# pfnet-research/superpixel-align

Measured on AMD Instinct MI355X. Metric: images/sec superpixel-align labelling (1024x2048), higher is better.
Workload: dtype f32 as 2 x f16 planes, f32 accumulate

## Files before the change

superpixel-align_amd/csrc/spa_common.h:

```cpp
#pragma once
#include <hip/hip_runtime.h>
#include <stdint.h>
#include <stdio.h>
#include <string.h>

#include "../../include/spalign.h"

#define SPA_WAVE 64

void spa_set_error(const char *fmt, ...);

#define SPA_HIP(call)                                                                  \
    do {                                                                               \
        hipError_t e_ = (call);                                                        \
        if (e_ != hipSuccess) {                                                        \
            spa_set_error("%s failed: %s (%s:%d)", #call, hipGetErrorString(e_),      \
                          __FILE__, __LINE__);                                         \
            return SPA_ERR_HIP;                                                        \
        }                                                                              \
    } while (0)

#define SPA_ARG(cond)                                                                  \
    do {                                                                               \
        if (!(cond)) {                                                                 \
// ... 40 lines not shown
    WS_FZ_KEYS,
    WS_FZ_VALS,
    WS_FZ_STATE,
    WS_FZ_TMP,
    WS_STEM_WPACK,
    WS_ZERO_LINE,
    WS_RESIZE_TAB,
    WS_RESIZE_TMP,
    WS_RNG_STATE,
    WS_RNG_RING,
    WS_RNG_JBUF,
    WS_RNG_JOFF,
    WS_RUNS,
    WS_DEBUG,
    WS_SEGNET_BNPART,
    WS_SEGNET_WROT,
    WS_SEGNET_WGRAD,
    WS_SEGNET_WBF16,
    WS_SEGNET_WF16X3,
    WS_SEGNET_AMAX,
    WS_SEGNET_BNRED,
    WS_PNG_ROWS,
    WS_JPEG_INTERVALS,
    WS_COUNT
};

enum {
    PROF_RGB2LAB = 0, PROF_SLIC_ASSIGN, PROF_SLIC_UPDATE, PROF_CONNECT, PROF_STATS,
    PROF_CELL_WEIGHTS, PROF_POOL_MEAN, PROF_POOL_ANCHOR, PROF_KMEANS, PROF_PAINT,
    PROF_DRN_STEM, PROF_DRN_BIAS_ACT, PROF_DRN_CONV, PROF_DRN_CONV32, PROF_DRN_GEMM32, PROF_DRN_GEMM32_N, PROF_WINO_IN, PROF_WINO_OUT, PROF_DRN_GEMM16, PROF_DRN_GEMM16_N, PROF_DRN_CONV16, PROF_DRN_CONV16_128, PROF_DRN_CONV16_256, PROF_DRN_CONV16_1X1, PROF_DRN_CONV16_FRONT, PROF_DRN_CONV_LIGHT, PROF_SLOTS
};

struct spa_ctx {
    int device;
    int n_cu;
    uint32_t *d_status;
    unsigned status_takes;
    void *ws[WS_COUNT];
    size_t ws_bytes[WS_COUNT];
    int prof_on;
    hipEvent_t *prof_ev[PROF_SLOTS];
    int prof_cap[PROF_SLOTS], prof_used[PROF_SLOTS];
    hipStream_t aux[2];
    hipEvent_t ev_fork, ev_join[2];
    int aux_ready;
    int km_attr_done[2];
    int conn_attr_done;
    int conn_claim_ready;
    size_t conn_claim_bytes;
    int upd_wg_per_cu, upd_wg_per_cu8;
    int slic_force_general;
    int zero_line_ready, conv_attr_done, conv32_attr_done, fz_attr_done, gemm16_attr_done, gemm16s_attr_done, gemm16p_attr_done, nprng_attr_done;
    int rng_seeded;
    int ws_generation;
    int dbg_slic_ldsx;
    int convp_on;
    int wino_operands;
    int convs2_on;
    int convs2_attr_done;
    int rs_key[4], rs_ks[2];
};

#ifdef __HIPCC__
__device__ __forceinline__ unsigned spa_split16_pair(float x0, float x1, float sc, unsigned &l)
{
    unsigned h, lo;
    asm("v_fma_mixlo_f16 %0, %2, %4, 0 op_sel_hi:[0,0,0]\n\t"
        "v_fma_mixhi_f16 %0, %3, %4, 0 op_sel_hi:[0,0,0]\n\t"
        "v_fma_mixlo_f16 %1, %2, %4, -%0 op_sel_hi:[0,0,1]\n\t"
        "v_fma_mixhi_f16 %1, %3, %4, -%0 op_sel:[0,0,1] op_sel_hi:[0,0,1]"
        : "=&v"(h), "=&v"(lo) : "v"(x0), "v"(x1), "v"(sc));
    l = lo;
    return h;
}
#endif

int spa_aux_streams(spa_ctx *ctx);

void spa_prof_mark(spa_ctx *ctx, int slot, int end, hipStream_t s);
struct SpaProfScope {
    spa_ctx *c; int slot; hipStream_t s;
    SpaProfScope(spa_ctx *c_, int slot_, hipStream_t s_) : c(c_), slot(slot_), s(s_) { if (c->prof_on && slot >= 0) spa_prof_mark(c, slot, 0, s); }
    ~SpaProfScope() { if (c->prof_on && slot >= 0) spa_prof_mark(c, slot, 1, s); }
};

int spa_ws_reserve(spa_ctx *ctx, int which, size_t bytes, void **out);
void spa_zero_word(void *word, hipStream_t s);

static inline hipStream_t spa_stream(void *s) { return (hipStream_t)s; }

__device__ __forceinline__ double spa_det_log_pos(double x)
{
    unsigned long long b = (unsigned long long)__double_as_longlong(x);
    int e = (int)((b >> 52) & 0x7ff) - 1023;
    b = (b & 0x000fffffffffffffULL) | 0x3ff0000000000000ULL;
    double m = __longlong_as_double((long long)b);
    if (m > 1.4142135623730951) { m = m * 0.5; e += 1; }
    double s = (m - 1.0) / (m + 1.0);
    double z = s * s;
    double p = 1.0 / 25.0;
    p = p * z + 1.0 / 23.0;
    p = p * z + 1.0 / 21.0;
    p = p * z + 1.0 / 19.0;
    p = p * z + 1.0 / 17.0;
    p = p * z + 1.0 / 15.0;
    p = p * z + 1.0 / 13.0;
    p = p * z + 1.0 / 11.0;
    p = p * z + 1.0 / 9.0;
    p = p * z + 1.0 / 7.0;
    p = p * z + 1.0 / 5.0;
// ... 37 lines not shown
```

superpixel-align_amd/csrc/spa_convs2.hip:

```cpp
#include "spa_common.h"

typedef float s2_f4 __attribute__((ext_vector_type(4)));
typedef _Float16 s2_h8 __attribute__((ext_vector_type(8)));

#define S2_TW 32
#define S2_PW (2 * S2_TW + 1)

__device__ __forceinline__ void s2_lds_barrier()
{
    asm volatile("s_waitcnt lgkmcnt(0)\n\ts_barrier" ::: "memory");
}

template <int CIN> struct S2Geom {
    static constexpr int TH = CIN == 32 ? 4 : 2;
    static constexpr int PH = 2 * TH + 1;
    static constexpr int PITCH = 4 * CIN + 16;
    static constexpr int PATCH = PH * S2_PW * PITCH;
    static constexpr int NW = 8;
    static constexpr int NE = PH * S2_PW * (CIN / 4), NU = (NE + NW * 64 - 1) / (NW * 64);
    static constexpr int NS = CIN == 32 ? 0 : (NU < 9 ? NU : 9);
    static constexpr int LDS = PATCH + NS * NW * 1024;
    static_assert(LDS <= 160 * 1024 && PATCH % 16 == 0, "LDS of a CU");
};

template <int CIN, int NG, bool PROJ>
__global__ __launch_bounds__(S2Geom<CIN>::NW * 64) void k_conv3x3_s2_tile(const float *__restrict__ x, int B, int Hi, int Wi, int Ho, int Wo,
                                                                const unsigned short *__restrict__ wt2, const float *__restrict__ bias,
                                                                float inv_t, int relu, const unsigned *__restrict__ amax_in,
                                                                unsigned *__restrict__ amax_out, float *__restrict__ y,
                                                                float *__restrict__ y2)
{
    typedef S2Geom<CIN> G;
    constexpr int TH = G::TH, PITCH = G::PITCH, KC = CIN / 32, CS = 16 * NG;
    constexpr int NW = G::NW, S2_THREADS = NW * 64, NE = G::NE, NU = G::NU, NS = G::NS;
    constexpr bool LIGHT = CIN == 64;
    constexpr int NPH = NW / NG, ITER = TH / NPH;
    static_assert(TH % NPH == 0 && NPH * NG == NW, "rows per wave");
    extern __shared__ __attribute__((aligned(16))) char s2_patch[];
    const int tid = threadIdx.x, lane = tid & 63;
    const int wave = __builtin_amdgcn_readfirstlane(tid >> 6);
    const int frow = lane & 15, fk = lane >> 4;
    const int cg = wave % NG, ph = wave / NG;
    const int tiles_x = (Wo + S2_TW - 1) / S2_TW, tiles_y = (Ho + TH - 1) / TH;
    const int n_tiles = tiles_x * tiles_y * B;

    s2_h8 wh[9][KC], wl[9][KC], qh[KC], ql[KC];
    float4 bias_c, bias_p;
    {
        const unsigned short *wr = wt2 + (size_t)(cg * 16 + frow) * (9 * KC * 64) + 8 * fk;
#pragma unroll
        for (int tap = 0; tap < 9; ++tap)
#pragma unroll
            for (int kc = 0; kc < KC; ++kc) {
                wh[tap][kc] = *(const s2_h8 *)(wr + (tap * KC + kc) * 64);
                wl[tap][kc] = *(const s2_h8 *)(wr + (tap * KC + kc) * 64 + 32);
            }
        bias_c = bias_p = make_float4(0.f, 0.f, 0.f, 0.f);
        if (!LIGHT) bias_c = *(const float4 *)(bias + cg * 16 + 4 * fk);
        if (PROJ && !LIGHT) {
            const unsigned short *pr = wt2 + (size_t)(CS + cg * 16 + frow) * (9 * KC * 64) + 8 * fk;
#pragma unroll
// ... 16 lines not shown
    constexpr int Q = CIN / 4;
    float4 raw[NU - NS > 0 ? NU - NS : 1];
    char *const stage = s2_patch + G::PATCH + wave * 1024;
    auto patch_load = [&](int tile) {
        const int b = tile / (tiles_x * tiles_y), tr = tile - b * (tiles_x * tiles_y);
        const int ty0 = (tr / tiles_x) * TH, tx0 = (tr % tiles_x) * S2_TW;
        const float *src = x + (long long)b * Hi * Wi * CIN;
#pragma unroll
        for (int u = 0; u < NU; ++u) {
            int e = tid + u * S2_THREADS;
            e = e < NE ? e : NE - 1;
            const int pix = e / Q, q = e % Q;
            const int iy = pix / S2_PW, ix = pix - iy * S2_PW;
            const int gy = 2 * ty0 - 1 + iy, gx = 2 * tx0 - 1 + ix;
            const int cy = min(max(gy, 0), Hi - 1), cx = min(max(gx, 0), Wi - 1);
            const float *g = src + ((long long)cy * Wi + cx) * CIN + 4 * q;
            if (u < NS)
                __builtin_amdgcn_global_load_lds((const __attribute__((address_space(1))) void *)g,
                                                 (__attribute__((address_space(3))) void *)(stage + u * (NW * 1024)), 16, 0, 0);
            else raw[u - NS] = *(const float4 *)g;
        }
    };
    unsigned amx = 0;
    if ((int)blockIdx.x < n_tiles) patch_load(blockIdx.x);
    for (int tile = blockIdx.x; tile < n_tiles; tile += gridDim.x) {
        const int b = tile / (tiles_x * tiles_y), tr = tile - b * (tiles_x * tiles_y);
        const int ty0 = (tr / tiles_x) * TH, tx0 = (tr % tiles_x) * S2_TW;
        if (NS > 0) asm volatile("s_waitcnt vmcnt(0)" ::: "memory");
#pragma unroll
        for (int u = 0; u < NU; ++u) {
            const int e = tid + u * S2_THREADS;
            if (e >= NE) continue;
            const int pix = e / Q, q = e % Q;
            const int iy = pix / S2_PW, ix = pix - iy * S2_PW;
            const int gy = 2 * ty0 - 1 + iy, gx = 2 * tx0 - 1 + ix;
            const bool in = (unsigned)gy < (unsigned)Hi && (unsigned)gx < (unsigned)Wi;
            const float4 rv = u < NS ? *(const float4 *)(stage + u * (NW * 1024) + 16 * lane) : raw[u < NS ? 0 : u - NS];
            const float v0 = in ? rv.x : 0.f, v1 = in ? rv.y : 0.f, v2 = in ? rv.z : 0.f, v3 = in ? rv.w : 0.f;
            unsigned l01, l23;
            const unsigned h01 = spa_split16_pair(v0, v1, sc, l01);
            const unsigned h23 = spa_split16_pair(v2, v3, sc, l23);
            char *o = s2_patch + pix * PITCH + q * 8;
            *(uint2 *)o = make_uint2(h01, h23);
            *(uint2 *)(o + 2 * CIN) = make_uint2(l01, l23);
        }
        s2_lds_barrier();
        if (tile + (int)gridDim.x < n_tiles) patch_load(tile + (int)gridDim.x);
#pragma unroll 1
        for (int it = 0; it < ITER; ++it) {
            const int r = ph * ITER + it;
            const char *pb = s2_patch + ((2 * r) * S2_PW + 2 * frow) * PITCH + 16 * fk;
            s2_f4 c0 = {0.f, 0.f, 0.f, 0.f}, c1 = {0.f, 0.f, 0.f, 0.f}, p0 = {0.f, 0.f, 0.f, 0.f}, p1 = {0.f, 0.f, 0.f, 0.f};
            if (PROJ && LIGHT) {
                size_t off = (size_t)(CS + frow) * (9 * KC * 64) + 8 * fk + 4 * KC * 64;
                asm volatile("" : "+v"(off));
#pragma unroll
                for (int kc = 0; kc < KC; ++kc) {
                    const unsigned short *pr = wt2 + off + (size_t)(cg * 16) * (9 * KC * 64) + kc * 64;
                    qh[kc] = *(const s2_h8 *)pr;
                    ql[kc] = *(const s2_h8 *)(pr + 32);
                }
            }
#pragma unroll
            for (int dy = 0; dy < 3; ++dy)
#pragma unroll
                for (int kc = 0; kc < KC; ++kc)
#pragma unroll
                    for (int dx = 0; dx < 3; ++dx) {
                        const int tap = dy * 3 + dx;
                        const char *f = pb + (dy * S2_PW + dx) * PITCH + kc * 64;
// ... 24 lines not shown
                for (int hf = 0; hf < 2; ++hf) {
                    const int gx = tx0 + hf * 16 + frow;
                    if (gx >= Wo) continue;
                    const long long pix = ((long long)b * Ho + gy) * Wo + gx;
                    const s2_f4 a = hf ? c1 : c0;
                    if (LIGHT) {
                        bias_c = *(const float4 *)(bias + cg * 16 + 4 * fk);
                        if (PROJ) bias_p = *(const float4 *)(bias + CS + cg * 16 + 4 * fk);
                    }
                    float v0 = a[0] * unscale + bias_c.x, v1 = a[1] * unscale + bias_c.y, v2 = a[2] * unscale + bias_c.z, v3 = a[3] * unscale + bias_c.w;
                    if (relu) { v0 = fmaxf(v0, 0.f); v1 = fmaxf(v1, 0.f); v2 = fmaxf(v2, 0.f); v3 = fmaxf(v3, 0.f); }
                    *(float4 *)(y + pix * CS + cg * 16 + 4 * fk) = make_float4(v0, v1, v2, v3);
                    amx = max(max(amx, __float_as_uint(v0) & 0x7fffffffu), max(__float_as_uint(v1) & 0x7fffffffu,
                              max(__float_as_uint(v2) & 0x7fffffffu, __float_as_uint(v3) & 0x7fffffffu)));
                    if (PROJ) {
                        const s2_f4 p = hf ? p1 : p0;
                        *(float4 *)(y2 + pix * CS + cg * 16 + 4 * fk) = make_float4(p[0] * unscale + bias_p.x, p[1] * unscale + bias_p.y,
                                                                                    p[2] * unscale + bias_p.z, p[3] * unscale + bias_p.w);
                    }
                }
            }
        }
        s2_lds_barrier();
    }
    if (amax_out) {
        for (int o = 32; o > 0; o >>= 1) amx = max(amx, (unsigned)__shfl_xor((int)amx, o));
        if (lane == 0 && amx > *(volatile unsigned *)amax_out) atomicMax(amax_out, amx);
    }
}

template <int CIN, int NG, bool PROJ>
static int s2_tile_launch(spa_ctx *ctx, int bit, const float *x, int B, int Hi, int Wi, const void *wt2, float inv_t, const float *bias,
                          int relu, const void *amax_in, void *amax_out, float *y, float *y2, hipStream_t s)
{
    typedef S2Geom<CIN> G;
    constexpr int NW = G::NW;
    if (!(ctx->convs2_attr_done & bit)) {
        SPA_HIP(hipFuncSetAttribute((const void *)k_conv3x3_s2_tile<CIN, NG, PROJ>, hipFuncAttributeMaxDynamicSharedMemorySize, G::LDS));
        ctx->convs2_attr_done |= bit;
    }
    const int Ho = (Hi + 1) / 2, Wo = (Wi + 1) / 2;
    const long long n_tiles = (long long)((Wo + S2_TW - 1) / S2_TW) * ((Ho + G::TH - 1) / G::TH) * B;
    SPA_ARG(n_tiles < (1ll << 31));
    long long grid = ctx->n_cu;
    if (grid > n_tiles) grid = n_tiles;
    hipLaunchKernelGGL((k_conv3x3_s2_tile<CIN, NG, PROJ>), dim3((unsigned)grid), dim3(NW * 64), G::LDS, s, x, B, Hi, Wi, Ho, Wo,
                       (const unsigned short *)wt2, bias, inv_t, relu, (const unsigned *)amax_in, (unsigned *)amax_out, y, y2);
    SPA_LAUNCH_CHECK();
    return SPA_OK;
}

bool conv3x3_s2_tile_takes(int32_t Cin, int32_t Cout, int32_t csplit, const float *y2)
{
    if (Cin != 32 && Cin != 64) return false;
    if (y2) return (csplit == 64 || csplit == 128) && Cout == 2 * csplit;
    return csplit == 128 && Cout == 128;
}

int conv3x3_s2_tile_launch(spa_ctx *ctx, const float *x, int32_t B, int32_t Hi, int32_t Wi, int32_t Cin, const void *wt2, float inv_t,
                           int32_t csplit, const float *bias, int32_t relu, const void *amax_in, void *amax_out, float *y, float *y2,
                           hipStream_t s)
{
#define S2_GO(C, N, P, BIT) return s2_tile_launch<C, N, P>(ctx, BIT, x, B, Hi, Wi, wt2, inv_t, bias, relu, amax_in, amax_out, y, y2, s)
    if (y2) {
        if (Cin == 32 && csplit == 64) S2_GO(32, 4, true, 1);
        if (Cin == 32 && csplit == 128) S2_GO(32, 8, true, 2);
        if (Cin == 64 && csplit == 64) S2_GO(64, 4, true, 4);
        if (Cin == 64 && csplit == 128) S2_GO(64, 8, true, 8);
    } else {
        if (Cin == 32 && csplit == 128) S2_GO(32, 8, false, 16);
// ... 7 lines not shown
```

superpixel-align_amd/csrc/spa_ctx.hip:

```cpp
#include <math.h>
#include <stdarg.h>
#include <stdlib.h>

#include "spa_common.h"

static thread_local char g_err[512] = "";

void spa_set_error(const char *fmt, ...)
{
    va_list ap;
    va_start(ap, fmt);
    vsnprintf(g_err, sizeof(g_err), fmt, ap);
    va_end(ap);
}

extern "C" const char *spa_last_error(void) { return g_err; }
extern "C" int spa_version(void) { return 100; }

extern "C" int spa_ctx_create(int device, spa_ctx **out)
{
    SPA_ARG(out != nullptr);
    int n = 0;
    if (hipGetDeviceCount(&n) != hipSuccess || n <= 0) {
        spa_set_error("no HIP device visible: libspalign has no CPU fallback");
        return SPA_ERR_NOGPU;
    }
    if (device < 0) SPA_HIP(hipGetDevice(&device));
    SPA_ARG(device < n);
    SPA_HIP(hipSetDevice(device));
    hipDeviceProp_t prop;
    SPA_HIP(hipGetDeviceProperties(&prop, device));
    if (strncmp(prop.gcnArchName, "gfx950", 6) != 0) {
        spa_set_error("device %d is %s; libspalign is built for gfx950 (MI355X) only", device,
                      prop.gcnArchName);
        return SPA_ERR_NOGPU;
    }
    spa_ctx *ctx = (spa_ctx *)calloc(1, sizeof(spa_ctx));
    ctx->device = device;
    ctx->n_cu = prop.multiProcessorCount;
    if (const char *e = getenv("SPA_SLIC_GENERAL")) ctx->slic_force_general = atoi(e) != 0;
    ctx->convp_on = getenv("SPA_CONVP") ? atoi(getenv("SPA_CONVP")) != 0 : 1;
    ctx->convs2_on = 1;
    ctx->wino_operands = 2;
    SPA_HIP(hipMalloc((void **)&ctx->d_status, 32 * sizeof(uint32_t)));
    SPA_HIP(hipMemset(ctx->d_status, 0, 32 * sizeof(uint32_t)));
    *out = ctx;
    return SPA_OK;
}

extern "C" void spa_ctx_destroy(spa_ctx *ctx)
{
    if (!ctx) return;
    for (int i = 0; i < PROF_SLOTS; ++i) {
        for (int j = 0; j < ctx->prof_cap[i]; ++j) (void)hipEventDestroy(ctx->prof_ev[i][j]);
        free(ctx->prof_ev[i]);
    }
    for (int i = 0; i < WS_COUNT; ++i)
        if (ctx->ws[i]) (void)hipFree(ctx->ws[i]);
    if (ctx->d_status) (void)hipFree(ctx->d_status);
    if (ctx->aux_ready) {
        for (int i = 0; i < 2; ++i) { (void)hipStreamDestroy(ctx->aux[i]); (void)hipEventDestroy(ctx->ev_join[i]); }
        (void)hipEventDestroy(ctx->ev_fork);
    }
    free(ctx);
}

__global__ void k_zero_word(unsigned *w) { *w = 0u; }
void spa_zero_word(void *word, hipStream_t s) { hipLaunchKernelGGL(k_zero_word, dim3(1), dim3(1), 0, s, (unsigned *)word); }

int spa_ws_reserve(spa_ctx *ctx, int which, size_t bytes, void **out)
{
    if (bytes == 0) bytes = 16;
    if (ctx->ws_bytes[which] < bytes) {
        SPA_HIP(hipDeviceSynchronize());
        if (ctx->ws[which]) SPA_HIP(hipFree(ctx->ws[which]));
        ctx->ws[which] = nullptr;
        ctx->ws_bytes[which] = 0;
        size_t want = bytes + bytes / 8;
        SPA_HIP(hipMalloc(&ctx->ws[which], want));
        ctx->ws_bytes[which] = want;
        ++ctx->ws_generation;
    }
    *out = ctx->ws[which];
    return SPA_OK;
}

extern "C" int spa_status(spa_ctx *ctx, uint32_t *status_host, void *stream)
{
    SPA_ARG(ctx && status_host);
    hipStream_t s = spa_stream(stream);
    SPA_HIP(hipMemcpyAsync(status_host, ctx->d_status, sizeof(uint32_t), hipMemcpyDeviceToHost, s));
// ... 199 lines not shown
            const bool take = best[i] > dd[i];
            best[i] = take ? dd[i] : best[i];
            bl[i] = take ? jj : bl[i];
        }
        if (p0.x < 1e30f) acc0 = p0;
        if (p1.x < 1e30f) acc1 = p1;
    }
    float4 r = make_float4(best[0] + (float)bl[0], best[1] + (float)bl[1], best[2] + (float)bl[2], best[3] + (float)bl[3]);
    *(float4 *)(out + ((long long)blockIdx.x * 256 + tid) * 4) = r;
}

extern "C" int spa_debug_lds_probe(spa_ctx *ctx, float *out, int32_t n_wg, int32_t steps, int32_t mode, void *stream)
{
    SPA_ARG(ctx && out && n_wg > 0 && steps > 0 && steps <= 32 && mode >= 0 && mode <= 2);
    hipLaunchKernelGGL(k_debug_lds_probe, dim3((unsigned)n_wg), dim3(256), 0, spa_stream(stream), out, steps, mode, 0.731f);
    SPA_LAUNCH_CHECK();
    return SPA_OK;
}

extern "C" int spa_ws_generation(spa_ctx *ctx) { return ctx ? ctx->ws_generation : -1; }

extern "C" int spa_debug_set(spa_ctx *ctx, int32_t key, int32_t value)
{
    SPA_ARG(ctx && (key == 1 || key == 2 || key == 3 || key == 4) && (value == 0 || value == 1 || (key == 4 && value == 2)));
    if (key == 1) ctx->convp_on = value;
    else if (key == 4) ctx->wino_operands = value;
    else if (key == 3) ctx->convs2_on = value;
    else {
#ifdef SPA_DIAG
        ctx->dbg_slic_ldsx = value;
#else
        SPA_ARG(!"spa_debug_set key 2 (the reproducer variant of k_slic_assign) exists in diagnostic builds only: make EXTRA=-DSPA_DIAG");
#endif
    }
    return SPA_OK;
}

extern "C" int spa_debug_peek(spa_ctx *ctx, int which, size_t offset, size_t bytes, void *host)
{
    if (which == -1) which = WS_DEBUG;
    SPA_ARG(ctx && host && which >= 0 && which < WS_COUNT && offset + bytes <= ctx->ws_bytes[which]);
    SPA_HIP(hipDeviceSynchronize());
    SPA_HIP(hipMemcpy(host, (const char *)ctx->ws[which] + offset, bytes, hipMemcpyDeviceToHost));
    return SPA_OK;
}
```

superpixel-align_amd/csrc/spa_stem.hip:

```cpp
#include "spa_common.h"

#define ST_TH 16
#define ST_TW 32
#define ST_IH (ST_TH + 8)
#define ST_IW (ST_TW + 8)
#define ST_IPLANE (ST_IH * ST_IW + 8)
#define ST_LH (ST_TH + 2)
#define ST_LW (ST_TW + 2)
#define ST_LP (ST_LH * ST_LW)
#define ST_PS 17
#define ST_K0 148
#define ST_S0 (ST_K0 / 4)
#define ST_S1 (144 / 4)
#define ST_PF 8

typedef float stem_f4 __attribute__((ext_vector_type(4)));

__device__ __forceinline__ unsigned short stem_bf16(float f)
{
    const unsigned u = __float_as_uint(f);
    if ((u & 0x7fffffffu) > 0x7f800000u) return (unsigned short)((u >> 16) | 0x0040u);
    return (unsigned short)((u + 0x7fffu + ((u >> 16) & 1u)) >> 16);
}

// ... 306 lines not shown
        }
        stem_lds_barrier();
    }
}

typedef _Float16 stem_h8 __attribute__((ext_vector_type(8)));
#define SH_PW 48
#define SH_PLANE (ST_IH * SH_PW + 16)
#define SH_COPY (3 * SH_PLANE + 48)
#define SH_L0_PITCH 32
#define SH_IN_S0 4096.0f

__device__ __forceinline__ unsigned short stem_f16_bits(float f)
{
    const _Float16 h = (_Float16)f;
    return __builtin_bit_cast(unsigned short, h);
}
__device__ __forceinline__ float stem_f16_val(unsigned short b) { return (float)__builtin_bit_cast(_Float16, b); }

__global__ __launch_bounds__(256, 2) void k_drn_stem_d_f16x3(const float *__restrict__ xn, int B, int H, int W,
                                                             const unsigned short *__restrict__ wp,
                                                             const float *__restrict__ b0, const float *__restrict__ b1,
                                                             float *__restrict__ y, unsigned *__restrict__ amax_out,
                                                             float *__restrict__ y0)
{
    __shared__ __attribute__((aligned(16))) unsigned short in_h[2][SH_COPY], in_l[2][SH_COPY];
    unsigned amx = 0;
    __shared__ __attribute__((aligned(16))) unsigned short l0_s[ST_LP * SH_L0_PITCH + 64];
    const int tid = threadIdx.x, lane = tid & 63, wv = tid >> 6;
    const int m = lane & 15, g = lane >> 4;
    const long long npix = (long long)H * W;
    const int tiles_x = (W + ST_TW - 1) / ST_TW, tiles_y = (H + ST_TH - 1) / ST_TH;
    const int n_tiles = tiles_x * tiles_y * B;

    stem_h8 w0h[6], w0l[6], w1h[5], w1l[5];
#pragma unroll
    for (int s = 0; s < 6; ++s) {
        w0h[s] = *(const stem_h8 *)(wp + ((size_t)s * 64 + lane) * 8);
        w0l[s] = *(const stem_h8 *)(wp + ((size_t)(6 + s) * 64 + lane) * 8);
    }
#pragma unroll
    for (int s = 0; s < 5; ++s) {
        w1h[s] = *(const stem_h8 *)(wp + ((size_t)(12 + s) * 64 + lane) * 8);
        w1l[s] = *(const stem_h8 *)(wp + ((size_t)(17 + s) * 64 + lane) * 8);
    }
    const float *sc = (const float *)(wp + (size_t)22 * 64 * 8);
    const float unscale0 = sc[0], s1 = sc[1], unscale1 = sc[2];
    const float4 bias0 = *(const float4 *)(b0 + 4 * g), bias1 = *(const float4 *)(b1 + 4 * g);
// ... 17 lines not shown
    int eiy[NU], eix[NU], elds[NU];
#pragma unroll
    for (int u = 0; u < NU; ++u) {
        int e = tid + u * 256;
        const bool ok = e < NE;
        if (!ok) e = NE - 1;
        const int pix = e / 3, c = e - pix * 3;
        eiy[u] = pix / ST_IW; eix[u] = pix - eiy[u] * ST_IW;
        elds[u] = ok ? c * SH_PLANE + eiy[u] * SH_PW + eix[u] : -1;
        eix[u] = eix[u] * 4 + c;
    }
    auto patch_load = [&](int tile) {
        const int b = tile / (tiles_x * tiles_y), tr = tile - b * (tiles_x * tiles_y);
        const int ty0 = (tr / tiles_x) * ST_TH, tx0 = (tr % tiles_x) * ST_TW;
        const float *src = xn + (long long)b * npix * 3;
#pragma unroll
        for (int u = 0; u < NU; ++u) {
            const int gy = ty0 - 4 + eiy[u], gx = tx0 - 4 + (eix[u] >> 2);
            const int cy = min(max(gy, 0), H - 1), cx = min(max(gx, 0), W - 1);
            raw[u] = src[(unsigned)((cy * W + cx) * 3 + (eix[u] & 3))];
        }
    };
    for (int i = tid; i < SH_COPY; i += 256) { in_h[0][i] = 0; in_h[1][i] = 0; in_l[0][i] = 0; in_l[1][i] = 0; }
    if ((int)blockIdx.x < n_tiles) patch_load(blockIdx.x);
    __syncthreads();

    for (int tile = blockIdx.x; tile < n_tiles; tile += gridDim.x) {
        const int b = tile / (tiles_x * tiles_y), tr = tile - b * (tiles_x * tiles_y);
        const int ty0 = (tr / tiles_x) * ST_TH, tx0 = (tr % tiles_x) * ST_TW;
#pragma unroll
        for (int u = 0; u < NU; ++u) {
            const int ix = eix[u] >> 2;
            const int gy = ty0 - 4 + eiy[u], gx = tx0 - 4 + ix;
            const bool in = (unsigned)gy < (unsigned)H && (unsigned)gx < (unsigned)W;
            if (elds[u] >= 0) {
                const float v = in ? raw[u] * SH_IN_S0 : 0.0f;
                const unsigned short vh = stem_f16_bits(v);
                const unsigned short vl = stem_f16_bits(v - stem_f16_val(vh));
                in_h[0][elds[u]] = vh; in_l[0][elds[u]] = vl;
                if (ix >= 1) { in_h[1][elds[u] - 1] = vh; in_l[1][elds[u] - 1] = vl; }
            }
        }
        stem_lds_barrier();

        for (int t = wv; t < (ST_LP + 15) / 16; t += 4) {
            int p = t * 16 + m;
            if (p > ST_LP - 1) p = ST_LP - 1;
            const int py = p / ST_LW, px = p - py * ST_LW;
            const int boff = py * SH_PW + (px & ~1);
            const unsigned short *bh = in_h[px & 1] + boff, *bl = in_l[px & 1] + boff;
            stem_f4 acc = {0.0f, 0.0f, 0.0f, 0.0f};
#pragma unroll
            for (int s = 0; s < 6; ++s) {
                const uint32_t *qh = (const uint32_t *)(bh + goff[s]), *ql = (const uint32_t *)(bl + goff[s]);
                union { uint32_t u[4]; stem_h8 v; } fh, fl;
                fh.u[0] = qh[0]; fh.u[1] = qh[1]; fh.u[2] = qh[2]; fh.u[3] = qh[3];
                fl.u[0] = ql[0]; fl.u[1] = ql[1]; fl.u[2] = ql[2]; fl.u[3] = ql[3];
                acc = __builtin_amdgcn_mfma_f32_16x16x32_f16(w0l[s], fh.v, acc, 0, 0, 0);
                acc = __builtin_amdgcn_mfma_f32_16x16x32_f16(w0h[s], fl.v, acc, 0, 0, 0);
                acc = __builtin_amdgcn_mfma_f32_16x16x32_f16(w0h[s], fh.v, acc, 0, 0, 0);
            }
            const int q0 = t * 16 + m;
            if (q0 < ST_LP) {
                const int gy = ty0 - 1 + py, gx = tx0 - 1 + px;
                const bool in = gy >= 0 && gy < H && gx >= 0 && gx < W;
                float v[4] = {acc[0] * unscale0 + bias0.x, acc[1] * unscale0 + bias0.y, acc[2] * unscale0 + bias0.z, acc[3] * unscale0 + bias0.w};
                unsigned short vh[4], vl[4];
#pragma unroll
                for (int j = 0; j < 4; ++j) {
                    const float r = in ? fmaxf(v[j], 0.0f) * s1 : 0.0f;
                    vh[j] = stem_f16_bits(r);
                    vl[j] = stem_f16_bits(r - stem_f16_val(vh[j]));
                }
                if (y0 && in && py >= 1 && py <= ST_TH && px >= 1 && px <= ST_TW)
                    *(float4 *)(y0 + ((((long long)b * H + gy) * W + gx) * 16 + 4 * g)) =
                        make_float4(fmaxf(v[0], 0.0f), fmaxf(v[1], 0.0f), fmaxf(v[2], 0.0f), fmaxf(v[3], 0.0f));
                const int sw = (q0 << 2) & 16;
                unsigned short *o = l0_s + q0 * SH_L0_PITCH + 4 * g;
                *(uint2 *)(o + sw) = make_uint2((unsigned)vh[0] | ((unsigned)vh[1] << 16), (unsigned)vh[2] | ((unsigned)vh[3] << 16));
                *(uint2 *)(o + 16 - sw) = make_uint2((unsigned)vl[0] | ((unsigned)vl[1] << 16), (unsigned)vl[2] | ((unsigned)vl[3] << 16));
            }
        }
        stem_lds_barrier();
        if (tile + (int)gridDim.x < n_tiles) patch_load(tile + (int)gridDim.x);

        for (int t = wv; t < 32; t += 4) {
            const int row = t >> 1, col = (t & 1) * 16 + m;
            stem_f4 acc = {0.0f, 0.0f, 0.0f, 0.0f};
            const int qb = row * ST_LW + col;
#pragma unroll
            for (int s = 0; s < 5; ++s) {
                const int q = qb + l1off[s];
                const int sw = (q << 2) & 16;
                const unsigned short *lb = l0_s + q * SH_L0_PITCH + 8 * (g & 1);
                const stem_h8 fh = *(const stem_h8 *)(lb + sw);
                const stem_h8 fl = *(const stem_h8 *)(lb + 16 - sw);
                acc = __builtin_amdgcn_mfma_f32_16x16x32_f16(w1l[s], fh, acc, 0, 0, 0);
                acc = __builtin_amdgcn_mfma_f32_16x16x32_f16(w1h[s], fl, acc, 0, 0, 0);
                acc = __builtin_amdgcn_mfma_f32_16x16x32_f16(w1h[s], fh, acc, 0, 0, 0);
            }
            const int gy = ty0 + row, gx = tx0 + col;
            if (gy < H && gx < W) {
                const float4 o = make_float4(fmaxf(acc[0] * unscale1 + bias1.x, 0.0f), fmaxf(acc[1] * unscale1 + bias1.y, 0.0f),
                                             fmaxf(acc[2] * unscale1 + bias1.z, 0.0f), fmaxf(acc[3] * unscale1 + bias1.w, 0.0f));
                *(float4 *)(y + ((((long long)b * H + gy) * W + gx) * 16 + 4 * g)) = o;
                amx = max(amx, max(max(__float_as_uint(o.x), __float_as_uint(o.y)), max(__float_as_uint(o.z), __float_as_uint(o.w))));
            }
        }
        stem_lds_barrier();
    }
    if (amax_out) {
        for (int o = 32; o > 0; o >>= 1) amx = max(amx, (unsigned)__shfl_xor((int)amx, o));
        if (lane == 0 && amx > *(volatile unsigned *)amax_out) atomicMax(amax_out, amx);
    }
}

#define L2_TH 4
#define L2_TW 32
#define L2_PH (2 * L2_TH + 1)
#define L2_PW (2 * L2_TW + 1)
#define L2_PITCH 40

__global__ __launch_bounds__(256, 2) void k_drn_layer2_f16x3(const float *__restrict__ x, int B, int H, int W, int Ho, int Wo,
                                                             const unsigned short *__restrict__ wp, const float *__restrict__ bias,
                                                             float inv_t, const unsigned *__restrict__ amax_in,
                                                             unsigned *__restrict__ amax_out, float *__restrict__ y)
{
    __shared__ __attribute__((aligned(16))) unsigned short patch[L2_PH * L2_PW * L2_PITCH + 64];
    const int tid = threadIdx.x, lane = tid & 63, wv = tid >> 6;
    const int m = lane & 15, g = lane >> 4;
    const int tiles_x = (Wo + L2_TW - 1) / L2_TW, tiles_y = (Ho + L2_TH - 1) / L2_TH;
    const int n_tiles = tiles_x * tiles_y * B;
    stem_h8 wh[2][5], wl[2][5];
#pragma unroll
    for (int ct = 0; ct < 2; ++ct)
#pragma unroll
        for (int s = 0; s < 5; ++s) {
            wh[ct][s] = *(const stem_h8 *)(wp + ((size_t)((ct * 2 + 0) * 5 + s) * 64 + lane) * 8);
            wl[ct][s] = *(const stem_h8 *)(wp + ((size_t)((ct * 2 + 1) * 5 + s) * 64 + lane) * 8);
        }
    float sc, unscale;
    {
        const unsigned bits = *amax_in;
        int e = (int)(bits >> 23) - 127;
        e = bits == 0u ? 0 : (e < -100 ? -100 : (e > 100 ? 100 : e));
        sc = __uint_as_float((unsigned)(127 + 14 - e) << 23);
        unscale = __uint_as_float((unsigned)(127 - 14 + e) << 23) * inv_t;
    }
    const float4 bias_lo = *(const float4 *)(bias + 4 * g), bias_hi = *(const float4 *)(bias + 16 + 4 * g);
    int toff[5];
#pragma unroll
// ... 6 lines not shown
    float4 raw[NU];
    int epix[NU], eq[NU];
#pragma unroll
    for (int u = 0; u < NU; ++u) {
        int e = tid + u * 256;
        if (e >= NE) e = -1;
        epix[u] = e < 0 ? -1 : e >> 2;
        eq[u] = e & 3;
    }
    auto patch_load = [&](int tile) {
        const int b = tile / (tiles_x * tiles_y), tr = tile - b * (tiles_x * tiles_y);
        const int ty0 = (tr / tiles_x) * L2_TH, tx0 = (tr % tiles_x) * L2_TW;
        const float *src = x + (long long)b * H * W * 16;
#pragma unroll
        for (int u = 0; u < NU; ++u) {
            const int pix = epix[u] < 0 ? 0 : epix[u];
            const int iy = pix / L2_PW, ix = pix - iy * L2_PW;
            const int gy = 2 * ty0 - 1 + iy, gx = 2 * tx0 - 1 + ix;
            const int cy = min(max(gy, 0), H - 1), cx = min(max(gx, 0), W - 1);
            raw[u] = *(const float4 *)(src + ((long long)cy * W + cx) * 16 + 4 * eq[u]);
        }
    };
    unsigned amx = 0;
    if ((int)blockIdx.x < n_tiles) patch_load(blockIdx.x);
    for (int tile = blockIdx.x; tile < n_tiles; tile += gridDim.x) {
        const int b = tile / (tiles_x * tiles_y), tr = tile - b * (tiles_x * tiles_y);
        const int ty0 = (tr / tiles_x) * L2_TH, tx0 = (tr % tiles_x) * L2_TW;
#pragma unroll
        for (int u = 0; u < NU; ++u) {
            if (epix[u] < 0) continue;
            const int iy = epix[u] / L2_PW, ix = epix[u] - iy * L2_PW;
            const int gy = 2 * ty0 - 1 + iy, gx = 2 * tx0 - 1 + ix;
            const bool in = (unsigned)gy < (unsigned)H && (unsigned)gx < (unsigned)W;
            const float v[4] = {in ? raw[u].x * sc : 0.f, in ? raw[u].y * sc : 0.f, in ? raw[u].z * sc : 0.f, in ? raw[u].w * sc : 0.f};
            unsigned short vh[4], vl[4];
#pragma unroll
            for (int j = 0; j < 4; ++j) { vh[j] = stem_f16_bits(v[j]); vl[j] = stem_f16_bits(v[j] - stem_f16_val(vh[j])); }
            unsigned short *o = patch + epix[u] * L2_PITCH + 4 * eq[u];
            *(uint2 *)o = make_uint2((unsigned)vh[0] | ((unsigned)vh[1] << 16), (unsigned)vh[2] | ((unsigned)vh[3] << 16));
            *(uint2 *)(o + 16) = make_uint2((unsigned)vl[0] | ((unsigned)vl[1] << 16), (unsigned)vl[2] | ((unsigned)vl[3] << 16));
        }
        stem_lds_barrier();
        if (tile + (int)gridDim.x < n_tiles) patch_load(tile + (int)gridDim.x);
        for (int t = wv; t < (L2_TH * L2_TW) / 16; t += 4) {
            const int row = t >> 1, col = (t & 1) * 16 + m;
            const unsigned short *pb = patch + ((2 * row) * L2_PW + 2 * col) * L2_PITCH;
            stem_f4 a0 = {0.f, 0.f, 0.f, 0.f}, a1 = {0.f, 0.f, 0.f, 0.f};
#pragma unroll
            for (int s = 0; s < 5; ++s) {
                const stem_h8 fh = *(const stem_h8 *)(pb + toff[s]);
                const stem_h8 fl = *(const stem_h8 *)(pb + toff[s] + 16);
                a0 = __builtin_amdgcn_mfma_f32_16x16x32_f16(wl[0][s], fh, a0, 0, 0, 0);
                a1 = __builtin_amdgcn_mfma_f32_16x16x32_f16(wl[1][s], fh, a1, 0, 0, 0);
                a0 = __builtin_amdgcn_mfma_f32_16x16x32_f16(wh[0][s], fl, a0, 0, 0, 0);
                a1 = __builtin_amdgcn_mfma_f32_16x16x32_f16(wh[1][s], fl, a1, 0, 0, 0);
                a0 = __builtin_amdgcn_mfma_f32_16x16x32_f16(wh[0][s], fh, a0, 0, 0, 0);
                a1 = __builtin_amdgcn_mfma_f32_16x16x32_f16(wh[1][s], fh, a1, 0, 0, 0);
            }
            const int gy = ty0 + row, gx = tx0 + col;
            if (gy < Ho && gx < Wo) {
                const float4 o0 = make_float4(fmaxf(a0[0] * unscale + bias_lo.x, 0.f), fmaxf(a0[1] * unscale + bias_lo.y, 0.f),
                                              fmaxf(a0[2] * unscale + bias_lo.z, 0.f), fmaxf(a0[3] * unscale + bias_lo.w, 0.f));
                const float4 o1 = make_float4(fmaxf(a1[0] * unscale + bias_hi.x, 0.f), fmaxf(a1[1] * unscale + bias_hi.y, 0.f),
                                              fmaxf(a1[2] * unscale + bias_hi.z, 0.f), fmaxf(a1[3] * unscale + bias_hi.w, 0.f));
                float *o = y + (((long long)b * Ho + gy) * Wo + gx) * 32 + 4 * g;
                *(float4 *)o = o0;
                *(float4 *)(o + 16) = o1;
                amx = max(amx, max(max(__float_as_uint(o0.x), __float_as_uint(o0.y)), max(__float_as_uint(o0.z), __float_as_uint(o0.w))));
                amx = max(amx, max(max(__float_as_uint(o1.x), __float_as_uint(o1.y)), max(__float_as_uint(o1.z), __float_as_uint(o1.w))));
            }
        }
        stem_lds_barrier();
    }
    if (amax_out) {
        for (int o = 32; o > 0; o >>= 1) amx = max(amx, (unsigned)__shfl_xor((int)amx, o));
        if (lane == 0 && amx > *(volatile unsigned *)amax_out) atomicMax(amax_out, amx);
    }
}

extern "C" int spa_drn_layer2_f16s(spa_ctx *ctx, const float *x, int32_t B, int32_t H, int32_t W, const void *wp, float inv_t,
                                   const float *bias, const void *amax_in, void *amax_out, float *y, void *stream)
{
    SPA_ARG(ctx && x && wp && bias && amax_in && y && B > 0 && H > 0 && W > 0 && inv_t > 0.f);
    SPA_ARG((((uintptr_t)x | (uintptr_t)wp | (uintptr_t)bias | (uintptr_t)y) & 15) == 0);
    hipStream_t s = spa_stream(stream);
    if (amax_out) spa_zero_word(amax_out, s);
    const int Ho = (H + 1) / 2, Wo = (W + 1) / 2;
    const long long n_tiles = (long long)((Wo + L2_TW - 1) / L2_TW) * ((Ho + L2_TH - 1) / L2_TH) * B;
    SPA_ARG(n_tiles < (1ll << 31));
    SpaProfScope prof_(ctx, PROF_DRN_CONV16_FRONT, s);
    long long grid = 3ll * ctx->n_cu;
    if (grid > n_tiles) grid = n_tiles;
    hipLaunchKernelGGL(k_drn_layer2_f16x3, dim3((unsigned)grid), dim3(256), 0, s, x, B, H, W, Ho, Wo, (const unsigned short *)wp, bias,
                       inv_t, (const unsigned *)amax_in, (unsigned *)amax_out, y);
    SPA_LAUNCH_CHECK();
    return SPA_OK;
}

__global__ __launch_bounds__(256) void k_drn_layer2_f32(const float *__restrict__ x, int B, int H, int W, int Ho, int Wo,
                                                       const float4 *__restrict__ w9, const float *__restrict__ bias, float *__restrict__ y)
{
    __shared__ float4 lw[9 * 16 * 8];
    for (int i = threadIdx.x; i < 9 * 16 * 8; i += 256) lw[i] = w9[i];
    __syncthreads();
    const long long id = (long long)blockIdx.x * 256 + threadIdx.x;
    if (id >= (long long)B * Ho * Wo) return;
    const int xo = (int)(id % Wo);
    const long long t = id / Wo;
    const int yo = (int)(t % Ho), b = (int)(t / Ho);
    typedef float l2f2 __attribute__((ext_vector_type(2)));
    l2f2 acc[16];
#pragma unroll
    for (int n = 0; n < 16; ++n) acc[n] = (l2f2){bias[2 * n], bias[2 * n + 1]};
    for (int tap = 0; tap < 9; ++tap) {
        const int yy = 2 * yo - 1 + tap / 3, xx = 2 * xo - 1 + tap % 3;
        if (yy < 0 || yy >= H || xx < 0 || xx >= W) continue;
        const float4 *px = (const float4 *)(x + (((long long)b * H + yy) * W + xx) * 16);
// ... 155 lines not shown
        if ((rc = spa_ws_reserve(ctx, WS_STEM_WPACK, (size_t)11 * 64 * 8 * 2, (void **)&wp)) != SPA_OK) return rc;
        hipLaunchKernelGGL(k_stem_pack_bf16, dim3(11), dim3(64), 0, spa_stream(stream), w0, w1, wp);
        unsigned short *xb = (unsigned short *)xn_scratch;
        if (!xb && (rc = spa_ws_reserve(ctx, WS_STEM_IN, (size_t)B * H * W * 3 * sizeof(float), (void **)&xb)) != SPA_OK) return rc;
        if ((rc = spa_drn_normalise(ctx, x, B, H, W, xb, 1, mean3_host, std3_host, stream)) != SPA_OK) return rc;
        hipLaunchKernelGGL(k_drn_stem_d_bf16, dim3((unsigned)grid), dim3(256), 0, spa_stream(stream), (const unsigned short *)xb, B,
                           H, W, (const unsigned short *)wp, b0, (const unsigned short *)(wp + 6 * 64 * 8), b1,
                           (unsigned short *)y, (unsigned short *)y0);
        SPA_LAUNCH_CHECK();
        return SPA_OK;
    }
    float *xn = xn_scratch;
    if (!xn) rc = spa_ws_reserve(ctx, WS_STEM_IN, (size_t)B * H * W * 3 * sizeof(float), (void **)&xn);
    if (rc != SPA_OK) return rc;
    rc = spa_drn_normalise(ctx, x, B, H, W, xn, 0, mean3_host, std3_host, stream);
    if (rc != SPA_OK) return rc;
    if (out_dtype == 2) {
        if (amax_out) spa_zero_word(amax_out, spa_stream(stream));
        unsigned short *wp;
        if ((rc = spa_ws_reserve(ctx, WS_STEM_WPACK, (size_t)22 * 64 * 8 * 2 + 16, (void **)&wp)) != SPA_OK) return rc;
        hipLaunchKernelGGL(k_stem_pack_f16, dim3(23), dim3(64), 0, spa_stream(stream), w0, b0, w1, wp);
        long long g2 = 2ll * ctx->n_cu;
        if (g2 > n_tiles) g2 = n_tiles;
        hipLaunchKernelGGL(k_drn_stem_d_f16x3, dim3((unsigned)g2), dim3(256), 0, spa_stream(stream), (const float *)xn, B, H, W,
                           (const unsigned short *)wp, b0, b1, (float *)y, (unsigned *)amax_out, y0);
        SPA_LAUNCH_CHECK();
        return SPA_OK;
    }
    hipLaunchKernelGGL(k_drn_stem_d, dim3((unsigned)grid), dim3(256), 0, spa_stream(stream), (const float *)xn, B, H, W,
                       w0, b0, w1, b1, y, (int)out_dtype);
    SPA_LAUNCH_CHECK();
    return SPA_OK;
}
```

superpixel-align_amd/drn.py:

```python
import collections
import gc
import math
import os
from functools import partial

import numpy as np
import torch
import torch.nn as nn
import torch.nn.functional as F

IMAGENET_MEAN = (0.485, 0.456, 0.406)
IMAGENET_STD = (0.229, 0.224, 0.225)
CHAINER_BN_EPS = 2e-5

_PLANS = {
    'drn_c_26': ('C', (1, 1, 2, 2, 2, 2, 1, 1)),
    'drn_d_22': ('D', (1, 1, 2, 2, 2, 2, 1, 1)),
}
_CHANNELS = (16, 32, 64, 128, 256, 512, 512, 512)


def _conv(cin, cout, k, stride=1, dilation=1):
    pad = dilation * (k // 2)
    return nn.Conv2d(cin, cout, k, stride=stride, padding=pad, dilation=dilation, bias=False)
# ... 46 lines not shown
        for i in range(3):
            c[i] += v[i]


def _graph_wanted(x):
    mode = os.environ.get('SPA_DRN_GRAPH', '')
    if mode == '0' or not x.is_cuda:
        return False
    if mode == '1':
        return True
    return x.shape[0] * x.shape[2] * x.shape[3] <= int(os.environ.get('SPA_DRN_GRAPH_PIXELS', str(4 << 20)))


F32, BF16 = torch.float32, torch.bfloat16
Flags = collections.namedtuple('Flags', 'split_gemm own_conv own_conv32 winograd bf16_light wino_min_cin debug')
Layer = collections.namedtuple('Layer', 'cin cout k stride dilation folded families')
Call = collections.namedtuple('Call', 'dtype B H W gpu layout residual relu')


def _flags():
    E, eng = _EPILOGUE, _EPILOGUE['engine']
    return Flags(E['split_gemm'], E['own_conv'], E['own_conv32'], E['winograd'], os.environ.get('SPA_BF16_LIGHT', '1') != '0',
                 int(os.environ.get('SPA_WINO_MIN_CIN', '256')),
                 None if eng is None else (eng.debug_get(1, 1), eng.debug_get(3, 1), eng.debug_get(4, 2)))


def _nhwc(*tensors):
    return all(t is None or t.is_contiguous(memory_format=torch.channels_last) for t in tensors)


def _layer(conv, bn, holder=None):
    return Layer(conv.in_channels, conv.out_channels, conv.kernel_size[0], conv.stride[0], conv.dilation[0],
                 isinstance(bn, nn.Identity) and conv.bias is not None, tuple(getattr(holder or conv, '_spa_ops', ())))


def _call(x, residual, relu):
    return Call(x.dtype, x.shape[0], x.shape[2], x.shape[3], _EPILOGUE['engine'] is not None and x.is_cuda, _nhwc(x, residual),
                residual is not None, relu)


def _row_fills(W, bn):
    return -(-W // bn) * bn <= 1.25 * W


def _out(n, stride):
    return -(-n // stride)

# ... 676 lines not shown
```

Measured before the change: 443.7.

## Replace static tile striding with atomic work-stealing queue in front conv kernels

```diff
diff --git a/superpixel-align_amd/csrc/spa_common.h b/superpixel-align_amd/csrc/spa_common.h
--- a/superpixel-align_amd/csrc/spa_common.h
+++ b/superpixel-align_amd/csrc/spa_common.h
@@ -86,6 +86,7 @@
     WS_SEGNET_BNRED,
     WS_PNG_ROWS,
     WS_JPEG_INTERVALS,
+    WS_TILE_QUEUE,
     WS_COUNT
 };
 
@@ -122,6 +123,8 @@
     int wino_operands;
     int convs2_on;
     int convs2_attr_done;
+    int tile_queue_on;
+    unsigned tile_queue_launches;
     int rs_key[4], rs_ks[2];
 };
 
@@ -137,6 +140,11 @@
     l = lo;
     return h;
 }
+
+__device__ __forceinline__ unsigned spa_tile_claim(unsigned *counter, unsigned chunk = 1)
+{
+    return gridDim.x + chunk * __hip_atomic_fetch_add(counter, 1u, __ATOMIC_RELAXED, __HIP_MEMORY_SCOPE_AGENT);
+}
 #endif
 
 int spa_aux_streams(spa_ctx *ctx);
@@ -150,6 +158,7 @@
 
 int spa_ws_reserve(spa_ctx *ctx, int which, size_t bytes, void **out);
 void spa_zero_word(void *word, hipStream_t s);
+int spa_tile_queue(spa_ctx *ctx, hipStream_t s, unsigned **counter);
 
 static inline hipStream_t spa_stream(void *s) { return (hipStream_t)s; }
 
diff --git a/superpixel-align_amd/csrc/spa_convs2.hip b/superpixel-align_amd/csrc/spa_convs2.hip
--- a/superpixel-align_amd/csrc/spa_convs2.hip
+++ b/superpixel-align_amd/csrc/spa_convs2.hip
@@ -28,7 +28,7 @@
                                                                 const unsigned short *__restrict__ wt2, const float *__restrict__ bias,
                                                                 float inv_t, int relu, const unsigned *__restrict__ amax_in,
                                                                 unsigned *__restrict__ amax_out, float *__restrict__ y,
-                                                                float *__restrict__ y2)
+                                                                float *__restrict__ y2, unsigned *__restrict__ tq)
 {
     typedef S2Geom<CIN> G;
     constexpr int TH = G::TH, PITCH = G::PITCH, KC = CIN / 32, CS = 16 * NG;
@@ -37,6 +37,7 @@
     constexpr int NPH = NW / NG, ITER = TH / NPH;
     static_assert(TH % NPH == 0 && NPH * NG == NW, "rows per wave");
     extern __shared__ __attribute__((aligned(16))) char s2_patch[];
+    __shared__ unsigned tq_next;
     const int tid = threadIdx.x, lane = tid & 63;
     const int wave = __builtin_amdgcn_readfirstlane(tid >> 6);
     const int frow = lane & 15, fk = lane >> 4;
@@ -99,8 +100,13 @@
         }
     };
     unsigned amx = 0;
-    if ((int)blockIdx.x < n_tiles) patch_load(blockIdx.x);
-    for (int tile = blockIdx.x; tile < n_tiles; tile += gridDim.x) {
+    unsigned claim = 0;
+    int tile = blockIdx.x;
+    if (tile < n_tiles) {
+        if (tq && tid == 0) claim = spa_tile_claim(tq);
+        patch_load(tile);
+    }
+    while (tile < n_tiles) {
         const int b = tile / (tiles_x * tiles_y), tr = tile - b * (tiles_x * tiles_y);
         const int ty0 = (tr / tiles_x) * TH, tx0 = (tr % tiles_x) * S2_TW;
         if (NS > 0) asm volatile("s_waitcnt vmcnt(0)" ::: "memory");
@@ -121,8 +127,13 @@
             *(uint2 *)o = make_uint2(h01, h23);
             *(uint2 *)(o + 2 * CIN) = make_uint2(l01, l23);
         }
+        if (tq && tid == 0) tq_next = claim;
         s2_lds_barrier();
-        if (tile + (int)gridDim.x < n_tiles) patch_load(tile + (int)gridDim.x);
+        const int nxt = tq ? (int)min(__builtin_amdgcn_readfirstlane(tq_next), (unsigned)n_tiles) : tile + (int)gridDim.x;
+        if (nxt < n_tiles) {
+            if (tq && tid == 0) claim = spa_tile_claim(tq);
+            patch_load(nxt);
+        }
 #pragma unroll 1
         for (int it = 0; it < ITER; ++it) {
             const int r = ph * ITER + it;
@@ -193,6 +204,7 @@
             }
         }
         s2_lds_barrier();
+        tile = nxt;
     }
     if (amax_out) {
         for (int o = 32; o > 0; o >>= 1) amx = max(amx, (unsigned)__shfl_xor((int)amx, o));
@@ -215,8 +227,11 @@
     SPA_ARG(n_tiles < (1ll << 31));
     long long grid = ctx->n_cu;
     if (grid > n_tiles) grid = n_tiles;
+    unsigned *tq;
+    int rc = spa_tile_queue(ctx, s, &tq);
+    if (rc != SPA_OK) return rc;
     hipLaunchKernelGGL((k_conv3x3_s2_tile<CIN, NG, PROJ>), dim3((unsigned)grid), dim3(NW * 64), G::LDS, s, x, B, Hi, Wi, Ho, Wo,
-                       (const unsigned short *)wt2, bias, inv_t, relu, (const unsigned *)amax_in, (unsigned *)amax_out, y, y2);
+                       (const unsigned short *)wt2, bias, inv_t, relu, (const unsigned *)amax_in, (unsigned *)amax_out, y, y2, tq);
     SPA_LAUNCH_CHECK();
     return SPA_OK;
 }
diff --git a/superpixel-align_amd/csrc/spa_ctx.hip b/superpixel-align_amd/csrc/spa_ctx.hip
--- a/superpixel-align_amd/csrc/spa_ctx.hip
+++ b/superpixel-align_amd/csrc/spa_ctx.hip
@@ -41,6 +41,7 @@
     if (const char *e = getenv("SPA_SLIC_GENERAL")) ctx->slic_force_general = atoi(e) != 0;
     ctx->convp_on = getenv("SPA_CONVP") ? atoi(getenv("SPA_CONVP")) != 0 : 1;
     ctx->convs2_on = 1;
+    ctx->tile_queue_on = getenv("SPA_TILE_QUEUE") ? atoi(getenv("SPA_TILE_QUEUE")) != 0 : 1;
     ctx->wino_operands = 2;
     SPA_HIP(hipMalloc((void **)&ctx->d_status, 32 * sizeof(uint32_t)));
     SPA_HIP(hipMemset(ctx->d_status, 0, 32 * sizeof(uint32_t)));
@@ -67,6 +68,18 @@
 
 __global__ void k_zero_word(unsigned *w) { *w = 0u; }
 void spa_zero_word(void *word, hipStream_t s) { hipLaunchKernelGGL(k_zero_word, dim3(1), dim3(1), 0, s, (unsigned *)word); }
+
+int spa_tile_queue(spa_ctx *ctx, hipStream_t s, unsigned **counter)
+{
+    *counter = nullptr;
+    if (!ctx->tile_queue_on) return SPA_OK;
+    char *ring;
+    int rc = spa_ws_reserve(ctx, WS_TILE_QUEUE, 64 * 64, (void **)&ring);
+    if (rc != SPA_OK) return rc;
+    *counter = (unsigned *)(ring + 64 * (ctx->tile_queue_launches++ & 63));
+    spa_zero_word(*counter, s);
+    return SPA_OK;
+}
 
 int spa_ws_reserve(spa_ctx *ctx, int which, size_t bytes, void **out)
 {
@@ -312,8 +325,9 @@
 
 extern "C" int spa_debug_set(spa_ctx *ctx, int32_t key, int32_t value)
 {
-    SPA_ARG(ctx && (key == 1 || key == 2 || key == 3 || key == 4) && (value == 0 || value == 1 || (key == 4 && value == 2)));
+    SPA_ARG(ctx && key >= 1 && key <= 5 && (value == 0 || value == 1 || (key == 4 && value == 2)));
     if (key == 1) ctx->convp_on = value;
+    else if (key == 5) ctx->tile_queue_on = value;
     else if (key == 4) ctx->wino_operands = value;
     else if (key == 3) ctx->convs2_on = value;
     else {
diff --git a/superpixel-align_amd/csrc/spa_stem.hip b/superpixel-align_amd/csrc/spa_stem.hip
--- a/superpixel-align_amd/csrc/spa_stem.hip
+++ b/superpixel-align_amd/csrc/spa_stem.hip
@@ -352,8 +352,9 @@
                                                              const unsigned short *__restrict__ wp,
                                                              const float *__restrict__ b0, const float *__restrict__ b1,
                                                              float *__restrict__ y, unsigned *__restrict__ amax_out,
-                                                             float *__restrict__ y0)
-{
+                                                             float *__restrict__ y0, unsigned *__restrict__ tq, int tq_chunk)
+{
+    __shared__ unsigned tq_next;
     __shared__ __attribute__((aligned(16))) unsigned short in_h[2][SH_COPY], in_l[2][SH_COPY];
     unsigned amx = 0;
     __shared__ __attribute__((aligned(16))) unsigned short l0_s[ST_LP * SH_L0_PITCH + 64];
@@ -417,10 +418,16 @@
         }
     };
     for (int i = tid; i < SH_COPY; i += 256) { in_h[0][i] = 0; in_h[1][i] = 0; in_l[0][i] = 0; in_l[1][i] = 0; }
-    if ((int)blockIdx.x < n_tiles) patch_load(blockIdx.x);
+    unsigned claim = 0;
+    int left = 0;
+    int tile = blockIdx.x;
+    if (tile < n_tiles) {
+        if (tq && tid == 0) claim = spa_tile_claim(tq, tq_chunk);
+        patch_load(tile);
+    }
     __syncthreads();
 
-    for (int tile = blockIdx.x; tile < n_tiles; tile += gridDim.x) {
+    while (tile < n_tiles) {
         const int b = tile / (tiles_x * tiles_y), tr = tile - b * (tiles_x * tiles_y);
         const int ty0 = (tr / tiles_x) * ST_TH, tx0 = (tr % tiles_x) * ST_TW;
 #pragma unroll
@@ -436,6 +443,7 @@
                 if (ix >= 1) { in_h[1][elds[u] - 1] = vh; in_l[1][elds[u] - 1] = vl; }
             }
         }
+        if (tq && tid == 0) tq_next = claim;
         stem_lds_barrier();
 
         for (int t = wv; t < (ST_LP + 15) / 16; t += 4) {
@@ -477,7 +485,14 @@
             }
         }
         stem_lds_barrier();
-        if (tile + (int)gridDim.x < n_tiles) patch_load(tile + (int)gridDim.x);
+        int nxt = tile + (int)gridDim.x;
+        if (tq && left > 0) { nxt = tile + 1; --left; }
+        else if (tq) {
+            nxt = (int)min(__builtin_amdgcn_readfirstlane(tq_next), (unsigned)n_tiles);
+            left = tq_chunk - 1;
+            if (tid == 0 && nxt < n_tiles) claim = spa_tile_claim(tq, tq_chunk);
+        }
+        if (nxt < n_tiles) patch_load(nxt);
 
         for (int t = wv; t < 32; t += 4) {
             const int row = t >> 1, col = (t & 1) * 16 + m;
@@ -503,6 +518,7 @@
             }
         }
         stem_lds_barrier();
+        tile = nxt;
     }
     if (amax_out) {
         for (int o = 32; o > 0; o >>= 1) amx = max(amx, (unsigned)__shfl_xor((int)amx, o));
@@ -519,9 +535,11 @@
 __global__ __launch_bounds__(256, 2) void k_drn_layer2_f16x3(const float *__restrict__ x, int B, int H, int W, int Ho, int Wo,
                                                              const unsigned short *__restrict__ wp, const float *__restrict__ bias,
                                                              float inv_t, const unsigned *__restrict__ amax_in,
-                                                             unsigned *__restrict__ amax_out, float *__restrict__ y)
+                                                             unsigned *__restrict__ amax_out, float *__restrict__ y,
+                                                             unsigned *__restrict__ tq, int tq_chunk)
 {
     __shared__ __attribute__((aligned(16))) unsigned short patch[L2_PH * L2_PW * L2_PITCH + 64];
+    __shared__ unsigned tq_next;
     const int tid = threadIdx.x, lane = tid & 63, wv = tid >> 6;
     const int m = lane & 15, g = lane >> 4;
     const int tiles_x = (Wo + L2_TW - 1) / L2_TW, tiles_y = (Ho + L2_TH - 1) / L2_TH;
@@ -574,8 +592,14 @@
         }
     };
     unsigned amx = 0;
-    if ((int)blockIdx.x < n_tiles) patch_load(blockIdx.x);
-    for (int tile = blockIdx.x; tile < n_tiles; tile += gridDim.x) {
+    unsigned claim = 0;
+    int left = 0;
+    int tile = blockIdx.x;
+    if (tile < n_tiles) {
+        if (tq && tid == 0) claim = spa_tile_claim(tq, tq_chunk);
+        patch_load(tile);
+    }
+    while (tile < n_tiles) {
         const int b = tile / (tiles_x * tiles_y), tr = tile - b * (tiles_x * tiles_y);
         const int ty0 = (tr / tiles_x) * L2_TH, tx0 = (tr % tiles_x) * L2_TW;
 #pragma unroll
@@ -592,8 +616,16 @@
             *(uint2 *)o = make_uint2((unsigned)vh[0] | ((unsigned)vh[1] << 16), (unsigned)vh[2] | ((unsigned)vh[3] << 16));
             *(uint2 *)(o + 16) = make_uint2((unsigned)vl[0] | ((unsigned)vl[1] << 16), (unsigned)vl[2] | ((unsigned)vl[3] << 16));
         }
+        if (tq && tid == 0) tq_next = claim;
         stem_lds_barrier();
-        if (tile + (int)gridDim.x < n_tiles) patch_load(tile + (int)gridDim.x);
+        int nxt = tile + (int)gridDim.x;
+        if (tq && left > 0) { nxt = tile + 1; --left; }
+        else if (tq) {
+            nxt = (int)min(__builtin_amdgcn_readfirstlane(tq_next), (unsigned)n_tiles);
+            left = tq_chunk - 1;
+            if (tid == 0 && nxt < n_tiles) claim = spa_tile_claim(tq, tq_chunk);
+        }
+        if (nxt < n_tiles) patch_load(nxt);
         for (int t = wv; t < (L2_TH * L2_TW) / 16; t += 4) {
             const int row = t >> 1, col = (t & 1) * 16 + m;
             const unsigned short *pb = patch + ((2 * row) * L2_PW + 2 * col) * L2_PITCH;
@@ -623,6 +655,7 @@
             }
         }
         stem_lds_barrier();
+        tile = nxt;
     }
     if (amax_out) {
         for (int o = 32; o > 0; o >>= 1) amx = max(amx, (unsigned)__shfl_xor((int)amx, o));
@@ -643,8 +676,12 @@
     SpaProfScope prof_(ctx, PROF_DRN_CONV16_FRONT, s);
     long long grid = 3ll * ctx->n_cu;
     if (grid > n_tiles) grid = n_tiles;
+    unsigned *tq;
+    int rc = spa_tile_queue(ctx, s, &tq);
+    if (rc != SPA_OK) return rc;
+    const int tq_chunk = 4;
     hipLaunchKernelGGL(k_drn_layer2_f16x3, dim3((unsigned)grid), dim3(256), 0, s, x, B, H, W, Ho, Wo, (const unsigned short *)wp, bias,
-                       inv_t, (const unsigned *)amax_in, (unsigned *)amax_out, y);
+                       inv_t, (const unsigned *)amax_in, (unsigned *)amax_out, y, tq, tq_chunk);
     SPA_LAUNCH_CHECK();
     return SPA_OK;
 }
@@ -846,8 +883,10 @@
         hipLaunchKernelGGL(k_stem_pack_f16, dim3(23), dim3(64), 0, spa_stream(stream), w0, b0, w1, wp);
         long long g2 = 2ll * ctx->n_cu;
         if (g2 > n_tiles) g2 = n_tiles;
+        unsigned *tq;
+        if ((rc = spa_tile_queue(ctx, spa_stream(stream), &tq)) != SPA_OK) return rc;
         hipLaunchKernelGGL(k_drn_stem_d_f16x3, dim3((unsigned)g2), dim3(256), 0, spa_stream(stream), (const float *)xn, B, H, W,
-                           (const unsigned short *)wp, b0, b1, (float *)y, (unsigned *)amax_out, y0);
+                           (const unsigned short *)wp, b0, b1, (float *)y, (unsigned *)amax_out, y0, tq, 4);
         SPA_LAUNCH_CHECK();
         return SPA_OK;
     }
diff --git a/superpixel-align_amd/drn.py b/superpixel-align_amd/drn.py
--- a/superpixel-align_amd/drn.py
+++ b/superpixel-align_amd/drn.py
@@ -92,7 +92,7 @@
     E, eng = _EPILOGUE, _EPILOGUE['engine']
     return Flags(E['split_gemm'], E['own_conv'], E['own_conv32'], E['winograd'], os.environ.get('SPA_BF16_LIGHT', '1') != '0',
                  int(os.environ.get('SPA_WINO_MIN_CIN', '256')),
-                 None if eng is None else (eng.debug_get(1, 1), eng.debug_get(3, 1), eng.debug_get(4, 2)))
+                 None if eng is None else (eng.debug_get(1, 1), eng.debug_get(3, 1), eng.debug_get(4, 2), eng.debug_get(5, 1)))
 
 
 def _nhwc(*tensors):
```

Result: slower. 439.1 (-1.0%).
